# olga24912/lodestar

Hardware: AMD Instinct MI355X
Metric: verified signature sets/sec (node) (higher is better)
Workload: dtype u32/u64 (28-bit-limb Montgomery integer arithmetic); 1 GPU; C2 gossip attestation flood: 16384 single-pubkey sets per GPU, 1 set per batchable job; pk_mode=device table, sig_encoding=compressed 96 B, distinct_messages=16384, group_sets=1024, group_policy=0, inflight=32, slots=3, hw_queues=4, merge_sets=131072, pipeline_depth=3, parallelism=shard-by-job x1 (in-process devices), no collective

## Files before the change

### lodestar_amd/csrc/curve.hpp

```cpp
#pragma once
#include "tower.hpp"

BLS_HD fp F_add(const fp& a, const fp& b) { return fp_add(a, b); }
BLS_HD fp F_sub(const fp& a, const fp& b) { return fp_sub(a, b); }
BLS_HD fp F_mul(const fp& a, const fp& b) { return fp_mul(a, b); }
BLS_HD fp F_sqr(const fp& a) { return fp_sqr(a); }
BLS_HD fp F_dbl(const fp& a) { return fp_dbl(a); }
BLS_HD fp F_neg(const fp& a) { return fp_neg(a); }
BLS_HD bool F_is_zero(const fp& a) { return fp_is_zero(a); }
BLS_HD fp F_select(bool c, const fp& a, const fp& b) { return fp_select(c, a, b); }
BLS_HD fp F_add_nr(const fp& a, const fp& b) { return fp_add_nr(a, b); }
BLS_HD fp F_add_sq(const fp& a, const fp& b) { return fp_add_nr(a, b); }
BLS_HD fp2 F_add(const fp2& a, const fp2& b) { return fp2_add(a, b); }
BLS_HD fp2 F_sub(const fp2& a, const fp2& b) { return fp2_sub(a, b); }
BLS_HD fp2 F_mul(const fp2& a, const fp2& b) { return fp2_mul(a, b); }
BLS_HD fp2 F_sqr(const fp2& a) { return fp2_sqr(a); }
BLS_HD fp2 F_dbl(const fp2& a) { return fp2_dbl(a); }
BLS_HD fp2 F_neg(const fp2& a) { return fp2_neg(a); }
BLS_HD bool F_is_zero(const fp2& a) { return fp2_is_zero(a); }
BLS_HD fp2 F_select(bool c, const fp2& a, const fp2& b) { return fp2_select(c, a, b); }
BLS_HD fp2 F_add_nr(const fp2& a, const fp2& b) { return fp2_add_nr(a, b); }
BLS_HD fp2 F_add_sq(const fp2& a, const fp2& b) { return fp2_add_norm(a, b); }
template <int W, class F>
struct lt {
// ... 161 lines not shown
    if (F_is_zero(rr)) return jac_dbl(p);
    return jac_infinity<F>();
  }
  F HH = F_sqr(H);
  F I = F_dbl(F_dbl(HH));
  F J = F_mul(H, I);
  F V = F_mul(p.x, I);
  jac<F> r;
  r.x = F_sub(F_sub(F_sqr(rr), J), F_dbl(V));
  r.y = F_sub(F_mul(rr, F_sub(V, r.x)), F_dbl(F_mul(p.y, J)));
  r.z = F_sub(F_sub(F_sqr(F_add(p.z, H)), Z1Z1), HH);
  return r;
}
template <class F>
BLS_INL jac<F> jac_add_aff(const jac<F>& p, const aff<F>& q) {
  if constexpr (lazy_curve<F>::addaff)
    return jac_add_aff_lazy(p, q);
  else
    return jac_add_aff_eager(p, q);
}

template <class F>
BLS_INL jac<F> jac_add_lazy(const jac<F>& p, const jac<F>& q) {
  if (jac_is_inf(p)) return q;
  if (jac_is_inf(q)) return p;
  const F Z1Z1 = F_sqr(p.z);
  const F Z2Z2 = F_sqr(q.z);
  const F U1 = F_mul(p.x, Z2Z2);
  const F U2 = F_mul(q.x, Z1Z1);
  const F S1 = F_mul(p.y, F_mul(q.z, Z2Z2));
  const F S2 = F_mul(q.y, F_mul(p.z, Z1Z1));
  const F H = F_lc(L<1>(U2), L<-1>(U1));
  const F rr = F_lc(L<2>(S2), L<-2>(S1));
  if (F_is_zero(H)) {
    if (F_is_zero(rr)) return jac_dbl(p);
    return jac_infinity<F>();
  }
  const F I = F_sqr(F_add_sq(H, H));
  const F J = F_mul(H, I);
  const F V = F_mul(U1, I);
  const F R2 = F_sqr(rr);
  jac<F> r;
  r.x = F_lc(L<1>(R2), L<-1>(J), L<-2>(V));
  const F M = F_mul(rr, F_lc(L<3>(V), L<-1>(R2), L<1>(J)));
  const F N = F_mul(S1, J);
  r.y = F_lc(L<1>(M), L<-2>(N));
  r.z = F_mul(F_lc(L<1>(F_sqr(F_add_sq(p.z, q.z))), L<-1>(Z1Z1), L<-1>(Z2Z2)), H);
  return r;
}
template <class F>
BLS_INL jac<F> jac_add_eager(const jac<F>& p, const jac<F>& q) {
  if (jac_is_inf(p)) return q;
  if (jac_is_inf(q)) return p;
  F Z1Z1 = F_sqr(p.z);
  F Z2Z2 = F_sqr(q.z);
  F U1 = F_mul(p.x, Z2Z2);
  F U2 = F_mul(q.x, Z1Z1);
  F S1 = F_mul(p.y, F_mul(q.z, Z2Z2));
  F S2 = F_mul(q.y, F_mul(p.z, Z1Z1));
  F H = F_sub(U2, U1);
  F rr = F_dbl(F_sub(S2, S1));
  if (F_is_zero(H)) {
    if (F_is_zero(rr)) return jac_dbl(p);
    return jac_infinity<F>();
  }
  F I = F_sqr(F_dbl(H));
  F J = F_mul(H, I);
  F V = F_mul(U1, I);
  jac<F> r;
  r.x = F_sub(F_sub(F_sqr(rr), J), F_dbl(V));
  r.y = F_sub(F_mul(rr, F_sub(V, r.x)), F_dbl(F_mul(S1, J)));
  r.z = F_mul(F_sub(F_sub(F_sqr(F_add(p.z, q.z)), Z1Z1), Z2Z2), H);
  return r;
}
template <class F>
BLS_INL jac<F> jac_add(const jac<F>& p, const jac<F>& q) {
  if constexpr (lazy_curve<F>::add)
    return jac_add_lazy(p, q);
  else
    return jac_add_eager(p, q);
}

template <class F>
BLS_HDNI jac<F> jac_mul_u64(const aff<F>& P, uint64_t k) {
  jac<F> r = jac_infinity<F>();
  if (k == 0) return r;
  int top = 63;
  while (((k >> top) & 1ull) == 0) top--;
  r = jac_from_aff(P);
  for (int i = top - 1; i >= 0; i--) {
    r = jac_dbl(r);
    if ((k >> i) & 1ull) r = jac_add_aff(r, P);
  }
  return r;
}

template <class F>
BLS_HDNI jac<F> jac_mul_zabs(const jac<F>& P) {
  jac<F> r = P;
  for (int i = 62; i >= 0; i--) {
    r = jac_dbl(r);
    if ((BLS_Z_ABS >> i) & 1ull) r = jac_add(r, P);
  }
  return r;
}

template <class F, class LoadP>
BLS_INL jac<F> jac_mul_zabs_ld(LoadP loadP) {
  jac<F> r = loadP();
#pragma unroll 1
  for (int i = 62; i >= 0; i--) {
    r = jac_dbl(r);
    if ((BLS_Z_ABS >> i) & 1ull) r = jac_add(r, loadP());
  }
  return r;
}
template <class F, class LoadA>
BLS_INL jac<F> jac_mul_zabs_lda(LoadA loadA) {
  jac<F> r = jac_from_aff(loadA());
#pragma unroll 1
  for (int i = 62; i >= 0; i--) {
    r = jac_dbl(r);
    if ((BLS_Z_ABS >> i) & 1ull) r = jac_add_aff(r, loadA());
  }
  return r;
}

BLS_HDNI bool jac_to_aff(const g1j& p, g1a& out) {
  if (jac_is_inf(p)) return false;
  fp zi = fp_inv(p.z);
  fp zi2 = fp_sqr(zi);
  out.x = fp_mul(p.x, zi2);
  out.y = fp_mul(p.y, fp_mul(zi2, zi));
  return true;
}
BLS_HDNI bool jac_to_aff(const g2j& p, g2a& out) {
  if (jac_is_inf(p)) return false;
  fp2 zi = fp2_inv(p.z);
  fp2 zi2 = fp2_sqr(zi);
  out.x = fp2_mul(p.x, zi2);
  out.y = fp2_mul(p.y, fp2_mul(zi2, zi));
  return true;
}

template <class F>
BLS_FN bool jac_eq(const jac<F>& p, const jac<F>& q) {
  bool pi = jac_is_inf(p), qi = jac_is_inf(q);
  if (pi || qi) return pi && qi;
  F Z1Z1 = F_sqr(p.z), Z2Z2 = F_sqr(q.z);
  if (!F_is_zero(F_sub(F_mul(p.x, Z2Z2), F_mul(q.x, Z1Z1)))) return false;
  F a = F_mul(p.y, F_mul(q.z, Z2Z2));
  F b = F_mul(q.y, F_mul(p.z, Z1Z1));
  return F_is_zero(F_sub(a, b));
}

BLS_FN g2j g2_psi(const g2j& p) {
  g2j r;
  r.x = fp2_mul(fp2_conj(p.x), PSI_X);
  r.y = fp2_mul(fp2_conj(p.y), PSI_Y);
  r.z = fp2_conj(p.z);
  return r;
}
BLS_FN g2j g2_psi2(const g2j& p) {
  g2j r;
  r.x = fp2_mul(p.x, PSI2_X);
  r.y = fp2_mul(p.y, PSI2_Y);
  r.z = p.z;
  return r;
}

BLS_FN g1j endo_lambda(const g1j& p) {
  g1j r = p;
  r.x = fp_mul(p.x, G1_BETA);
  return r;
}
BLS_FN g2j endo_lambda(const g2j& p) { return jac_neg(g2_psi2(p)); }

BLS_HDNI bool g2_in_subgroup(const g2a& p) {
  g2j P = jac_from_aff(p);
  g2j zP = jac_neg(jac_mul_zabs(P));
  return jac_eq(g2_psi(P), zP);
}
template <class LoadA>
BLS_INL bool g2_in_subgroup_ld(LoadA loadA) {
  const g2j zP = jac_neg(jac_mul_zabs_lda<fp2>(loadA));
  return jac_eq(g2_psi(jac_from_aff(loadA())), zP);
}

BLS_HD bool g1_on_curve(const g1a& p) {
  return fp_eq(fp_sqr(p.y), fp_add(fp_mul(fp_sqr(p.x), p.x), FP_B1));
}
BLS_HD bool g2_on_curve(const g2a& p) {
  return fp2_eq(fp2_sqr(p.y), fp2_add(fp2_mul(fp2_sqr(p.x), p.x), FP2_B2));
}
```

### lodestar_amd/csrc/k_awr.hip

```cpp
#include "k_common.hpp"
#include "seg_sum.hpp"

BLS_INL int awr_point(const AwrBuffers& a, uint32_t k, g1j& P, bool& skip) {
  skip = false;
  g1a q;
  if (a.pk_bytes) {
    uint8_t raw[96];
    const uint4* src = reinterpret_cast<const uint4*>(a.pk_bytes + (size_t)k * 96);
#pragma unroll
    for (int c = 0; c < 6; c++) {
      const uint4 v = src[c];
      const uint32_t w[4] = {v.x, v.y, v.z, v.w};
#pragma unroll
      for (int j = 0; j < 16; j++) raw[16 * c + j] = (uint8_t)(w[j >> 2] >> (8 * (j & 3)));
    }
    bool inf = false;
    int st = pk_decode96(raw, q, inf);
    if (st == BLS_OK && inf) st = BLS_PK_IS_INFINITY;
    if (st != BLS_OK) return st;
  } else {
    const uint32_t idx = a.pk_index[k];
    if (idx >= a.pk_table_n) return BLS_DEVICE_ERROR;
    q = ld_pktab(a.pk_table, idx);
  }
  P = jac_from_aff(q);
  return BLS_OK;
}
BLS_INL int awr_point(const AwrBuffers& a, uint32_t k, g2j& P, bool& skip) {
  const int st = a.sig_status[k];
  skip = st == BLS_OK && (a.sig_flags[k] & SF_SIG_INF);
  if (st == BLS_OK && !skip) P = jac_from_aff(ld_g2a(a.sig_aff, a.n, k));
  return st;
}

template <class F>
BLS_INL void awr_strided(const AwrBuffers& a, uint32_t first, uint32_t last, uint32_t t, uint32_t L, uint32_t q,
                         jac<F>& acc, uint32_t& err_k, int& err) {
#pragma unroll 1
  for (uint32_t k = first + t; k < last; k += L) {
    jac<F> P;
    bool skip;
    const int st = awr_point(a, k, P, skip);
    if (st != BLS_OK) {
      if (err == 0) {
        err = st;
        err_k = k;
      }
      continue;
    }
    if (skip) continue;
    const uint32_t qq = opaque_u32(q);
    tab_st(a.tab, a.tab_n, qq, 8, acc);
    const jac<F> R = jac_mul_scalar_word(P, a.words[k], a.tab, a.tab_n, qq);
    acc = jac_add(tab_ld<F>(a.tab, a.tab_n, opaque_u32(q), 8), R);
  }
}

BLS_INL uint32_t* awr_sums(const AwrBuffers& a, const g1j*) { return a.sum_pk; }
BLS_INL uint32_t* awr_sums(const AwrBuffers& a, const g2j*) { return a.sum_sig; }
template <class F>
BLS_INL void awr_store(const AwrBuffers& a, uint32_t g, const jac<F>& acc, uint32_t err_k, int err) {
  constexpr int which = sizeof(F) == sizeof(fp) ? 0 : 1;
  uint32_t* o = awr_sums(a, (const jac<F>*)0);
  const uint32_t* s = reinterpret_cast<const uint32_t*>(&acc);
#pragma unroll
  for (int w = 0; w < (int)(sizeof(jac<F>) / 4); w++) o[(size_t)w * a.n_groups + g] = s[w];
  a.err_k[which * a.n_groups + g] = err_k;
  a.err_c[which * a.n_groups + g] = (int8_t)err;
}

template <class F, int L>
STAGE_KERNEL_W(1) void k_awr_sum(AwrBuffers a) {
  const uint32_t q = blockIdx.x * WAVE + threadIdx.x;
  const uint32_t t = q % L, g = q / L;
  const bool on = g < a.n_groups;
  const uint32_t first = on ? a.group_first[g] : 0, last = on ? a.group_first[g + 1] : 0;
  jac<F> acc = jac_infinity<F>();
  uint32_t my_err_k = 0xffffffffu;
  int my_err = 0;
  awr_strided<F>(a, first, last, t, L, q, acc, my_err_k, my_err);
  if constexpr (L == WAVE) {
    __shared__ uint32_t red[SEG_SLOTS * (sizeof(jac<F>) / 4)];
    __shared__ uint32_t err_k[WAVE];
    __shared__ int32_t err_c[WAVE];
    uint32_t bk;
    int bc;
    seg_wave_first_error(err_k, err_c, t, my_err_k, my_err, bk, bc);
    if (last - first > 1) seg_wave_tree(acc, red, t);
    my_err_k = bk;
    my_err = bc;
  } else {
    seg_butterfly<F, L>(acc, my_err_k, my_err);
  }
  if (on && t == 0) awr_store<F>(a, g, acc, my_err_k, my_err);
}

__global__ __launch_bounds__(WAVE) void k_awr_serialize(AwrBuffers a, uint8_t* out_pk, uint32_t out_pk_len,
                                                        uint8_t* out_sig, uint32_t out_sig_len, int8_t* status,
                                                        uint32_t* first_bad) {
  const uint32_t g = blockIdx.x * WAVE + threadIdx.x;
  if (g >= a.n_groups) return;
  const uint32_t kp = a.err_k[g], ks = a.err_k[a.n_groups + g];
  const bool key_first = kp <= ks;
  const uint32_t bad = key_first ? kp : ks;
  int st = key_first ? a.err_c[g] : a.err_c[a.n_groups + g];
  if (a.group_first[g + 1] == a.group_first[g]) st = BLS_EMPTY_AGGREGATE;
  uint8_t buf[192];
  for (int k = 0; k < 192; k++) buf[k] = 0;
  if (st == BLS_OK) {
    g1a p;
    if (!jac_to_aff(ld_g1j(a.sum_pk, a.n_groups, g), p)) {
      buf[0] = out_pk_len == 48 ? 0xc0 : 0x40;
    } else if (out_pk_len == 48) {
      g1a_compress(p, buf);
    } else {
      g1a_to_be96(p, buf);
    }
  }
  uint8_t* o = out_pk + (size_t)g * out_pk_len;
  for (uint32_t k = 0; k < out_pk_len; k++) o[k] = buf[k];
  for (int k = 0; k < 96; k++) buf[k] = 0;
  if (st == BLS_OK) {
    g2a s;
    if (!jac_to_aff(ld_g2j(a.sum_sig, a.n_groups, g), s)) {
      buf[0] = out_sig_len == 96 ? 0xc0 : 0x40;
    } else if (out_sig_len == 96) {
      g2a_compress(s, buf);
    } else {
      g2a_to_be192(s, buf);
    }
  }
  o = out_sig + (size_t)g * out_sig_len;
  for (uint32_t k = 0; k < out_sig_len; k++) o[k] = buf[k];
  status[g] = (int8_t)st;
  first_bad[g] = st == BLS_OK || st == BLS_EMPTY_AGGREGATE ? 0xffffffffu : bad;
}
// ... 32 lines not shown
```

### lodestar_amd/csrc/k_common.hpp

```cpp
#pragma once
#include <atomic>

#include "kernels.h"
#include "ops.hpp"
#include "fp2x.hpp"

#define WAVE 64
#if defined(__HIP_DEVICE_COMPILE__) && !BLS_INLINE_PRODUCTS && !BLS_FP2_CLASSIC
static_assert(WAVE <= BLS_FP2_LDS_LANES, "fp2_mul LDS slot");
static_assert(2 * WAVE <= BLS_FP2_LDS_LANES, "128-lane kernels (gt_wave.hpp, k_msm_bucket) and fp2_mul LDS slot");
#endif

#ifndef BLSGPU_WPE
#define BLSGPU_WPE 1
#endif
#define STAGE_KERNEL __global__ __launch_bounds__(WAVE) __attribute__((amdgpu_waves_per_eu(BLSGPU_WPE, BLSGPU_WPE)))
#define STAGE_KERNEL_W(w) __global__ __launch_bounds__(WAVE) __attribute__((amdgpu_waves_per_eu(w, w)))
#ifndef BLSGPU_WPE_PK
#define BLSGPU_WPE_PK BLSGPU_WPE
#endif
#ifndef BLSGPU_WPE_HPREP
#define BLSGPU_WPE_HPREP 1
#endif
#ifndef BLSGPU_WPE_MSM
#define BLSGPU_WPE_MSM BLSGPU_WPE
#endif
#ifndef BLSGPU_WPE_LINES
#define BLSGPU_WPE_LINES BLSGPU_WPE
#endif
#ifndef BLSGPU_WPE_ACC
#define BLSGPU_WPE_ACC BLSGPU_WPE
#endif
#ifndef BLSGPU_WPE_DEC
#define BLSGPU_WPE_DEC BLSGPU_WPE
#endif
#ifndef BLSGPU_WPE_HASH
#define BLSGPU_WPE_HASH BLSGPU_WPE
#endif
#ifndef BLSGPU_WPE_HMAP
#define BLSGPU_WPE_HMAP 2
#endif
#ifndef BLSGPU_WPE_GRP
#define BLSGPU_WPE_GRP BLSGPU_WPE
#endif

__device__ __forceinline__ uint32_t opaque_u32(uint32_t x) {
  asm volatile("" : "+v"(x));
  return x;
}

__device__ __forceinline__ fp ld_fp(const uint32_t* p, uint32_t n, uint32_t i, int w0) {
  fp r;
#pragma unroll
  for (int l = 0; l < BLS_NL; l++) r.l[l] = p[(size_t)(w0 + l) * n + i];
  return r;
}
__device__ __forceinline__ void st_fp(uint32_t* p, uint32_t n, uint32_t i, int w0, const fp& v) {
#pragma unroll
  for (int l = 0; l < BLS_NL; l++) p[(size_t)(w0 + l) * n + i] = v.l[l];
}
__device__ __forceinline__ fp2 ld_fp2(const uint32_t* p, uint32_t n, uint32_t i, int w0) {
  return fp2_make(ld_fp(p, n, i, w0), ld_fp(p, n, i, w0 + W_FP));
}
__device__ __forceinline__ void st_fp2(uint32_t* p, uint32_t n, uint32_t i, int w0, const fp2& v) {
  st_fp(p, n, i, w0, v.c0);
  st_fp(p, n, i, w0 + W_FP, v.c1);
}
__device__ __forceinline__ g2a ld_g2a(const uint32_t* p, uint32_t n, uint32_t i) {
  g2a r;
  r.x = ld_fp2(p, n, i, 0);
  r.y = ld_fp2(p, n, i, 2 * W_FP);
  return r;
}
__device__ __forceinline__ void st_g2a(uint32_t* p, uint32_t n, uint32_t i, const g2a& v) {
  st_fp2(p, n, i, 0, v.x);
  st_fp2(p, n, i, 2 * W_FP, v.y);
}
__device__ __forceinline__ g2j ld_g2j(const uint32_t* p, uint32_t n, uint32_t i) {
  g2j r;
  r.x = ld_fp2(p, n, i, 0);
  r.y = ld_fp2(p, n, i, 2 * W_FP);
  r.z = ld_fp2(p, n, i, 4 * W_FP);
  return r;
}
__device__ __forceinline__ void st_g2j(uint32_t* p, uint32_t n, uint32_t i, const g2j& v) {
  st_fp2(p, n, i, 0, v.x);
  st_fp2(p, n, i, 2 * W_FP, v.y);
  st_fp2(p, n, i, 4 * W_FP, v.z);
}
__device__ __forceinline__ g1a ld_g1a(const uint32_t* p, uint32_t n, uint32_t i) {
  g1a r;
  r.x = ld_fp(p, n, i, 0);
  r.y = ld_fp(p, n, i, W_FP);
  return r;
}
__device__ __forceinline__ void st_g1a(uint32_t* p, uint32_t n, uint32_t i, const g1a& v) {
  st_fp(p, n, i, 0, v.x);
  st_fp(p, n, i, W_FP, v.y);
}
__device__ __forceinline__ g1j ld_g1j(const uint32_t* p, uint32_t n, uint32_t i) {
  g1j r;
  r.x = ld_fp(p, n, i, 0);
// ... 55 lines not shown
  for (int s = 0; s < MILLER_STEPS; s++) {
    line3 L;
    if (!add_next) {
      miller_dbl_line(T, L);
      add_next = (BLS_Z_ABS >> bit) & 1ull;
      bit--;
    } else {
      miller_add_line(T, Q, L);
      add_next = false;
    }
    uint32_t* o = lines + (size_t)s * W_LINE * nm;
    st_fp2(o, nm, u, 0, L.l0);
    st_fp2(o, nm, u, 2 * W_FP, L.c1);
    st_fp2(o, nm, u, 4 * W_FP, L.c4);
  }
}

BLS_INL fp fp_shfl(const fp& x, int src) {
  fp r;
#pragma unroll
  for (int i = 0; i < BLS_NL; i++) r.l[i] = (uint32_t)__shfl((int)x.l[i], src);
  return r;
}
BLS_INL fp2 fp2_shfl(const fp2& x, int src) { return fp2_make(fp_shfl(x.c0, src), fp_shfl(x.c1, src)); }
BLS_INL fp fp_keep(bool c, const fp& a) { return fp_select(c, a, fp_zero()); }
#define ACC6_GROUPS (WAVE / 6)
BLS_INL g2j g2j_xlane(const g2j& p) {
  g2j r;
  r.x = fp2_xlane(p.x);
  r.y = fp2_xlane(p.y);
  r.z = fp2_xlane(p.z);
  return r;
}
__device__ __forceinline__ g1a ld_pktab(const uint32_t* tab, uint32_t idx) {
  const uint4* q = reinterpret_cast<const uint4*>(tab + (size_t)idx * W_PKTAB);
  uint32_t w[W_PKTAB];
#pragma unroll
  for (int k = 0; k < W_PKTAB / 4; k++) {
    uint4 v = q[k];
    w[4 * k] = v.x;
    w[4 * k + 1] = v.y;
    w[4 * k + 2] = v.z;
    w[4 * k + 3] = v.w;
  }
  g1a r;
#pragma unroll
  for (int l = 0; l < BLS_NL; l++) {
    r.x.l[l] = w[l];
    r.y.l[l] = w[BLS_NL + l];
  }
  return r;
}

template <class F>
__device__ jac<F> jac_mul_u64_j(const jac<F>& P, uint64_t k) {
  jac<F> r = jac_infinity<F>();
  if (k == 0) return r;
  int top = 63;
  while (((k >> top) & 1ull) == 0) top--;
  r = P;
  for (int i = top - 1; i >= 0; i--) {
    r = jac_dbl(r);
    if ((k >> i) & 1ull) r = jac_add(r, P);
  }
  return r;
}

template <class F>
__device__ __forceinline__ void tab_st(uint32_t* tab, uint32_t n, uint32_t i, int e, const jac<F>& v) {
  constexpr int WF = sizeof(F) / 4;
  const uint32_t* s = reinterpret_cast<const uint32_t*>(&v);
#pragma unroll
  for (int w = 0; w < 3 * WF; w++) tab[((size_t)e * 3 * WF + w) * n + i] = s[w];
}
template <class F>
__device__ __forceinline__ jac<F> tab_ld(const uint32_t* tab, uint32_t n, uint32_t i, int e) {
  constexpr int WF = sizeof(F) / 4;
  jac<F> v;
  uint32_t* d = reinterpret_cast<uint32_t*>(&v);
#pragma unroll
  for (int w = 0; w < 3 * WF; w++) d[w] = tab[((size_t)e * 3 * WF + w) * n + i];
  return v;
}
BLS_HD int scalar_word_digit(uint64_t w, int k, bool& neg) {
  const int d = 2 * (int)((w >> (4 * k)) & 15u) - 15;
  neg = d < 0;
  return (d < 0 ? -d : d) >> 1;
}
template <class F>
__device__ jac<F> jac_mul_scalar_word(const jac<F>& P, uint64_t w, uint32_t* tab, uint32_t n, uint32_t i) {
  const jac<F> P2 = jac_dbl(P);
  jac<F> t = P;
  tab_st(tab, n, i, 0, t);
#pragma unroll 1
  for (int e = 1; e < 8; e++) {
    t = jac_add(t, P2);
    tab_st(tab, n, i, e, t);
  }
  const uint32_t ii = opaque_u32(i);
  auto term = [&](int k, bool hi) {
    bool neg;
    const int e = scalar_word_digit(w, hi ? k + 8 : k, neg);
    jac<F> q = tab_ld<F>(tab, n, ii, e);
    if (hi) q = endo_lambda(q);
    return neg ? jac_neg(q) : q;
  };
  jac<F> r = jac_add(term(7, false), term(7, true));
#pragma unroll 1
  for (int k = 6; k >= 0; k--) {
    r = jac_dbl(jac_dbl(jac_dbl(jac_dbl(r))));
    r = jac_add(r, term(k, false));
    r = jac_add(r, term(k, true));
  }
  return r;
}

template <class F>
__device__ jac<F> jac_mul_words(const jac<F>& P, const uint32_t* k, int nw) {
  jac<F> r = jac_infinity<F>();
  for (int i = 32 * nw - 1; i >= 0; i--) {
    r = jac_dbl(r);
    if ((k[i >> 5] >> (i & 31)) & 1u) r = jac_add(r, P);
  }
  return r;
}


template <auto kernel>
inline size_t exclusive_cu_lds() {
  constexpr int kMaxDev = 64;
  static std::atomic<int64_t> cache[kMaxDev];
  int dev = 0;
  if (hipGetDevice(&dev) != hipSuccess || dev < 0 || dev >= kMaxDev) return 0;
  const int64_t c = cache[dev].load(std::memory_order_acquire);
  if (c) return (size_t)(c - 1);
  const size_t pad = [&]() -> size_t {
    int max_block = 0, per_cu = 0;
    if (hipDeviceGetAttribute(&max_block, hipDeviceAttributeMaxSharedMemoryPerBlock, dev) != hipSuccess) return 0;
    if (hipDeviceGetAttribute(&per_cu, hipDeviceAttributeMaxSharedMemoryPerMultiprocessor, dev) != hipSuccess)
      return 0;
    hipFuncAttributes a{};
    if (hipFuncGetAttributes(&a, reinterpret_cast<const void*>(kernel)) != hipSuccess) return 0;
    const size_t want = (size_t)per_cu - 8 * 1024;
    if (per_cu <= 0 || (size_t)max_block < want || a.sharedSizeBytes >= want) return 0;
    const size_t pad_b = want - a.sharedSizeBytes;
    if (hipFuncSetAttribute(reinterpret_cast<const void*>(kernel), hipFuncAttributeMaxDynamicSharedMemorySize,
                            (int)pad_b) != hipSuccess)
      return 0;
    return pad_b;
  }();
  cache[dev].store((int64_t)pad + 1, std::memory_order_release);
  return pad;
}
```

### lodestar_amd/csrc/k_pk.hip

```cpp
#include "k_common.hpp"
#include "pk_row.hpp"

static_assert(PK_ROW_WORDS == W_PKTAB, "pk_row.hpp restates the row width of kernels.h");

#ifndef BLSGPU_PK_AGG_GROUPS
#define BLSGPU_PK_AGG_GROUPS 1
#endif
__global__ __launch_bounds__(WAVE) void k_pk_aggregate(PipelineBuffers b, uint32_t n_sets) {
  __shared__ uint32_t red[WAVE * W_G1J];
  __shared__ uint32_t err_k[WAVE];
  __shared__ int32_t err_c[WAVE];
  if (blockIdx.x >= n_sets) return;
  const uint32_t set = b.agg_sets ? b.agg_sets[blockIdx.x] : blockIdx.x;
  uint32_t lane = threadIdx.x;
  int8_t* agg_status = b.status + 2 * b.n;
  const uint32_t first = b.set_pk_first[set], last = b.set_pk_first[set + 1];
  g1j acc = jac_infinity<fp>();
  uint32_t my_err_k = 0xffffffffu;
  int my_err = 0;
  for (uint32_t k = first + lane; k < last; k += WAVE) {
    g1a q;
    if (b.pk_bytes) {
      uint8_t raw[96];
      const uint8_t* src = b.pk_bytes + (size_t)k * 96;
// ... 93 lines not shown
      const int st = pk_decode96(raw, pt, inf);
      if (st != BLS_OK) {
        if (my_err == 0) {
          my_err = st;
          my_err_k = k;
        }
        continue;
      }
      if (inf) continue;
    } else {
      const uint32_t idx = b.pk_index[k];
      if (idx >= b.pk_table_n) {
        if (my_err == 0) {
          my_err = BLS_DEVICE_ERROR;
          my_err_k = k;
        }
        continue;
      }
      pt = ld_pktab(b.pk_table, idx);
    }
    acc = jac_add_aff(acc, pt);
  }
#pragma unroll 1
  for (int m = L / 2; m >= 1; m >>= 1) {
    g1j o;
    o.x = fp_shfl_xor(acc.x, m);
    o.y = fp_shfl_xor(acc.y, m);
    o.z = fp_shfl_xor(acc.z, m);
    const uint32_t ok = (uint32_t)__shfl_xor((int)my_err_k, m);
    const int oc = __shfl_xor(my_err, m);
    if (ok < my_err_k) {
      my_err_k = ok;
      my_err = oc;
    }
    acc = jac_add(acc, o);
  }
  if (on && t == 0) {
    b.status[2 * b.n + set] = (int8_t)my_err;
    st_g1j(b.pk_jac, b.n, set, acc);
  }
}

__device__ __forceinline__ int set_pubkey(const PipelineBuffers& b, uint32_t i, g1j& P) {
  const bool one = b.set_pk_first && b.pk_direct1 && b.set_pk_first[i + 1] - b.set_pk_first[i] == 1;
  if (one && !b.pk_bytes) {
    const uint32_t idx = b.pk_index[b.set_pk_first[i]];
    if (idx >= b.pk_table_n) return BLS_DEVICE_ERROR;
    P = jac_from_aff(ld_pktab(b.pk_table, idx));
    return BLS_OK;
  }
  if (b.pk_bytes && (!b.set_pk_first || one)) {
    uint8_t raw[96];
    const uint32_t k = b.set_pk_first ? b.set_pk_first[i] : i;
    const uint4* src = reinterpret_cast<const uint4*>(b.pk_bytes + (size_t)k * 96);
#pragma unroll
    for (int k = 0; k < 6; k++) {
      uint4 v = src[k];
      uint32_t w[4] = {v.x, v.y, v.z, v.w};
#pragma unroll
      for (int j = 0; j < 16; j++) raw[16 * k + j] = (uint8_t)(w[j >> 2] >> (8 * (j & 3)));
    }
    g1a a;
    bool inf = false;
    int st = pk_decode96(raw, a, inf);
    if (st == BLS_OK && inf) st = BLS_PK_IS_INFINITY;
    if (st == BLS_OK) P = jac_from_aff(a);
    return st;
  }
  if (b.set_pk_first[i + 1] == b.set_pk_first[i]) return BLS_EMPTY_AGGREGATE;
  const int st = b.status[2 * b.n + i];
  if (st) return st;
  P = ld_g1j(b.pk_jac, b.n, i);
  return jac_is_inf(P) ? BLS_PK_IS_INFINITY : BLS_OK;
}

STAGE_KERNEL_W(BLSGPU_WPE_PK) void k_pk_finish(PipelineBuffers b, uint32_t n_sets, int8_t* pk_status) {
  uint32_t i = blockIdx.x * WAVE + threadIdx.x;
  if (i >= n_sets) return;
  g1j P;
  int st = set_pubkey(b, i, P);
  g1j R = jac_infinity<fp>();
  if (st == BLS_OK) {
    const uint64_t w = b.scalars[i];
    R = (w == 0) ? P : jac_mul_scalar_word(P, w, b.scal_tab, b.n, i);
  }
  st_g1j(b.pk_jac, b.n, i, R);
  pk_status[i] = (int8_t)st;
}

STAGE_KERNEL void k_unit_aggregate(PipelineBuffers b) {
  uint32_t u = blockIdx.x * WAVE + threadIdx.x;
  if (u >= b.n_units) return;
  const uint32_t a = b.unit_set_first[u], e = b.unit_set_first[u + 1];
  g1a out;
  out.x = fp_zero();
  out.y = fp_zero();
  bool ok = false;
  if (e - a == 1) {
    const uint32_t i = b.unit_sets[a];
    if (b.include[i]) {
      out = ld_g1a(b.pk_aff, b.n, i);
      ok = true;
    }
  } else {
    g1j acc = jac_infinity<fp>();
    for (uint32_t k = a; k < e; k++) {
      const uint32_t i = b.unit_sets[k];
      if (b.include[i]) acc = jac_add_aff(acc, ld_g1a(b.pk_aff, b.n, i));
    }
    ok = jac_to_aff(acc, out);
  }
  st_g1a(b.unit_p, b.n, u, out);
  b.unit_ok[u] = ok ? 1 : 0;
}

__global__ __launch_bounds__(WAVE) void k_pk_serialize(PipelineBuffers b, uint32_t n_sets, uint8_t* out,
                                                       uint32_t out_len) {
  uint32_t i = blockIdx.x * WAVE + threadIdx.x;
  if (i >= n_sets) return;
  int st = b.set_pk_first[i + 1] == b.set_pk_first[i] ? BLS_EMPTY_AGGREGATE : b.status[2 * b.n + i];
  uint8_t buf[96];
  for (int k = 0; k < 96; k++) buf[k] = 0;
  if (st == BLS_OK) {
    g1a a;
    if (!jac_to_aff(ld_g1j(b.pk_jac, b.n, i), a)) {
      buf[0] = out_len == 48 ? 0xc0 : 0x40;
    } else if (out_len == 48) {
      g1a_compress(a, buf);
    } else {
      g1a_to_be96(a, buf);
    }
  }
  uint8_t* o = out + (size_t)i * out_len;
  for (uint32_t k = 0; k < out_len; k++) o[k] = buf[k];
  b.status[i] = (int8_t)st;
}

__global__ __launch_bounds__(WAVE) void k_key_validate(const uint8_t* pks, uint32_t n, uint32_t pk_len, uint32_t stride,
                                                       uint8_t* out96, int8_t* status) {
  uint32_t i = blockIdx.x * WAVE + threadIdx.x;
  if (i >= n) return;
  uint8_t raw[96];
  const uint8_t* src = pks + (size_t)i * stride;
  for (uint32_t k = 0; k < 96; k++) raw[k] = k < pk_len ? src[k] : 0;
  g1a a;
  const int st = pk_key_validate(raw, pk_len, a);
  uint8_t buf[96];
  for (int k = 0; k < 96; k++) buf[k] = 0;
  if (st == BLS_OK) g1a_to_be96(a, buf);
  if (out96)
    for (int k = 0; k < 96; k++) out96[(size_t)i * 96 + k] = buf[k];
  status[i] = (int8_t)st;
}

__global__ __launch_bounds__(WAVE) void k_pk_table_fill(const uint8_t* pk96, uint32_t n, uint32_t* table_dst,
                                                        int8_t* status) {
  uint32_t i = blockIdx.x * WAVE + threadIdx.x;
  if (i >= n) return;
  uint8_t raw[96];
  for (int k = 0; k < 96; k++) raw[k] = pk96[(size_t)i * 96 + k];
  g1a a;
  bool inf = false;
  int st = pk_decode96(raw, a, inf);
  if (st == BLS_OK && inf) st = BLS_PK_IS_INFINITY;
  uint32_t* dst = table_dst + (size_t)i * W_PKTAB;
  for (int l = 0; l < BLS_NL; l++) {
    dst[l] = st == BLS_OK ? a.x.l[l] : 0;
    dst[BLS_NL + l] = st == BLS_OK ? a.y.l[l] : 0;
  }
  dst[2 * BLS_NL] = 0;
  dst[2 * BLS_NL + 1] = 0;
  dst[2 * BLS_NL + 2] = 0;
  dst[2 * BLS_NL + 3] = 0;
  status[i] = (int8_t)st;
}

template <bool validate>
__global__ __launch_bounds__(WAVE) void k_pk_table_fill48(const uint8_t* pk48, uint32_t n, uint32_t* table_dst,
                                                          int8_t* status) {
  const uint32_t i = blockIdx.x * WAVE + threadIdx.x;
  if (i >= n) return;
  uint8_t raw[48];
  const uint4* src = reinterpret_cast<const uint4*>(pk48 + (size_t)i * 48);
#pragma unroll
  for (int k = 0; k < 3; k++) {
    const uint4 v = src[k];
    const uint32_t w[4] = {v.x, v.y, v.z, v.w};
#pragma unroll
    for (int j = 0; j < 16; j++) raw[16 * k + j] = (uint8_t)(w[j >> 2] >> (8 * (j & 3)));
  }
  uint32_t row[W_PKTAB];
  const int st = pk_row_from48<validate>(raw, row);
  uint4* dst = reinterpret_cast<uint4*>(table_dst + (size_t)i * W_PKTAB);
#pragma unroll
  for (int k = 0; k < W_PKTAB / 4; k++) dst[k] = make_uint4(row[4 * k], row[4 * k + 1], row[4 * k + 2], row[4 * k + 3]);
  status[i] = (int8_t)st;
}

__global__ __launch_bounds__(WAVE) void k_pk_table_read(const uint32_t* table, uint32_t first, uint32_t n, uint8_t* out,
                                                        uint32_t out_len) {
  const uint32_t i = blockIdx.x * WAVE + threadIdx.x;
  if (i >= n) return;
  const g1a a = ld_pktab(table, first + i);
  uint8_t buf[96];
  pk_point_to_bytes(a, out_len, buf);
  uint4* dst = reinterpret_cast<uint4*>(out + (size_t)i * out_len);
  const uint32_t quads = out_len / 16;
#pragma unroll
  for (uint32_t k = 0; k < 6; k++) {
    if (k >= quads) break;
    uint32_t w[4];
#pragma unroll
    for (int j = 0; j < 4; j++)
      w[j] = (uint32_t)buf[16 * k + 4 * j] | (uint32_t)buf[16 * k + 4 * j + 1] << 8 |
             (uint32_t)buf[16 * k + 4 * j + 2] << 16 | (uint32_t)buf[16 * k + 4 * j + 3] << 24;
    dst[k] = make_uint4(w[0], w[1], w[2], w[3]);
  }
}

static inline dim3 grid_for(uint32_t n) { return dim3((n + WAVE - 1) / WAVE); }

void launch_pk_aggregate(const PipelineBuffers& b, uint32_t n, hipStream_t s) {
  if (b.agg_sets) n = b.n_agg;
  if (!n) return;
  const uint32_t lanes = 1024 * WAVE;
  if ((uint64_t)n * 64 <= lanes || !BLSGPU_PK_AGG_GROUPS)
    hipLaunchKernelGGL(k_pk_aggregate, dim3(n), dim3(WAVE), 0, s, b, n);
  else if ((uint64_t)n * 32 <= 2 * lanes)
    hipLaunchKernelGGL(k_pk_aggregate_g<32>, dim3((n * 32 + WAVE - 1) / WAVE), dim3(WAVE), 0, s, b, n);
  else if ((uint64_t)n * 16 <= 2 * lanes)
    hipLaunchKernelGGL(k_pk_aggregate_g<16>, dim3((n * 16 + WAVE - 1) / WAVE), dim3(WAVE), 0, s, b, n);
  else
    hipLaunchKernelGGL(k_pk_aggregate_g<8>, dim3((n * 8 + WAVE - 1) / WAVE), dim3(WAVE), 0, s, b, n);
}
void launch_pk_finish(const PipelineBuffers& b, uint32_t n, hipStream_t s) {
  if (n) hipLaunchKernelGGL(k_pk_finish, grid_for(n), dim3(WAVE), 0, s, b, n, b.status + b.n);
}
void launch_unit_aggregate(const PipelineBuffers& b, hipStream_t s) {
  if (b.n_units) hipLaunchKernelGGL(k_unit_aggregate, grid_for(b.n_units), dim3(WAVE), 0, s, b);
}
void launch_pk_serialize(const PipelineBuffers& b, uint32_t n, uint8_t* out, uint32_t out_len, hipStream_t s) {
  if (n) hipLaunchKernelGGL(k_pk_serialize, grid_for(n), dim3(WAVE), 0, s, b, n, out, out_len);
}
void launch_key_validate(const uint8_t* pks, uint32_t n, uint32_t pk_len, uint32_t stride, uint8_t* out96,
                         int8_t* status, hipStream_t s) {
  if (n) hipLaunchKernelGGL(k_key_validate, grid_for(n), dim3(WAVE), 0, s, pks, n, pk_len, stride, out96, status);
}
void launch_pk_table_fill(const uint8_t* pk96, uint32_t n, uint32_t* table_dst, int8_t* status, hipStream_t s) {
  if (n) hipLaunchKernelGGL(k_pk_table_fill, grid_for(n), dim3(WAVE), 0, s, pk96, n, table_dst, status);
}
void launch_pk_table_fill48(const uint8_t* pk48, uint32_t n, uint32_t* table_dst, int8_t* status, bool validate,
                            hipStream_t s) {
  if (!n) return;
  if (validate)
    hipLaunchKernelGGL(k_pk_table_fill48<true>, grid_for(n), dim3(WAVE), 0, s, pk48, n, table_dst, status);
  else
    hipLaunchKernelGGL(k_pk_table_fill48<false>, grid_for(n), dim3(WAVE), 0, s, pk48, n, table_dst, status);
}
void launch_pk_table_read(const uint32_t* table, uint32_t first, uint32_t n, uint8_t* out, uint32_t out_len,
                          hipStream_t s) {
  if (n) hipLaunchKernelGGL(k_pk_table_read, grid_for(n), dim3(WAVE), 0, s, table, first, n, out, out_len);
}
```

### lodestar_amd/csrc/k_sig.hip

```cpp
#include "k_common.hpp"
#include "g2_coop.hpp"

#ifndef BLSGPU_SIG_PAIRS
#define BLSGPU_SIG_PAIRS 1
#endif
#ifndef BLSGPU_WPE_DEC0
#define BLSGPU_WPE_DEC0 2
#endif
#ifndef BLSGPU_WPE_SUB2
#define BLSGPU_WPE_SUB2 2
#endif
template <bool CHECK, int WPE>
__global__ __launch_bounds__(WAVE) __attribute__((amdgpu_waves_per_eu(WPE, WPE))) void k_sig_decode(
    PipelineBuffers b, uint32_t n_sets) {
  const bool check_group = CHECK;
  uint32_t i = blockIdx.x * WAVE + threadIdx.x;
  if (i >= n_sets) return;
  uint8_t raw[192];
  uint32_t len = b.sig_len[i];
  const uint8_t* src = b.sigs + (size_t)i * b.sig_stride;
  uint32_t cl = len == 96 || len == 192 ? len : 0;
  for (uint32_t k = 0; k < cl; k++) raw[k] = src[k];
  g2a p;
  bool inf = false;
  int st = sig_decode_point(raw, len, p, inf);
  if (st != BLS_OK || inf) {
    p.x = fp2_zero();
    p.y = fp2_zero();
  }
  st_g2a(b.sig_aff, b.n, i, p);
  if (check_group && st == BLS_OK && !inf &&
      !g2_in_subgroup_ld([&] { return ld_g2a(b.sig_aff, b.n, opaque_u32(i)); })) {
    st = BLS_POINT_NOT_IN_GROUP;
    p.x = fp2_zero();
    p.y = fp2_zero();
    st_g2a(b.sig_aff, b.n, i, p);
  }
  b.flags[i] = inf ? SF_SIG_INF : 0;
  b.status[i] = (int8_t)st;
}

STAGE_KERNEL_W(BLSGPU_WPE_SUB2) void k_sig_subgroup2(PipelineBuffers b, uint32_t n_sets) {
  const uint32_t q = blockIdx.x * WAVE + threadIdx.x, i = q >> 1, k = q & 1;
  if (i >= n_sets || b.status[i] != BLS_OK || (b.flags[i] & SF_SIG_INF)) return;
  auto ldP = [&] {
    const uint32_t ii = opaque_u32(i);
    aff<fp2x> a;
    a.x.v = ld_fp(b.sig_aff, b.n, ii, (int)(k * W_FP));
    a.y.v = ld_fp(b.sig_aff, b.n, ii, (int)((2 + k) * W_FP));
    return a;
  };
  const g2jx zP = jac_neg(jac_mul_zabs_lda<fp2x>(ldP));
  if (!jac_eq(g2_psi(jac_from_aff(ldP())), zP)) {
    st_fp(b.sig_aff, b.n, i, (int)(k * W_FP), fp_zero());
    st_fp(b.sig_aff, b.n, i, (int)((2 + k) * W_FP), fp_zero());
    if (k == 0) b.status[i] = (int8_t)BLS_POINT_NOT_IN_GROUP;
  }
}

STAGE_KERNEL void k_sig_scale(PipelineBuffers b, uint32_t n_sets, const uint32_t* list) {
  const uint32_t q = blockIdx.x * WAVE + threadIdx.x;
  if (q >= n_sets) return;
  const uint32_t i = list ? list[q] : q;
  g2j R = jac_infinity<fp2>();
  if (b.status[i] == BLS_OK && !(b.flags[i] & SF_SIG_INF)) {
    const g2a s = ld_g2a(b.sig_aff, b.n, i);
    const uint64_t w = b.scalars[i];
    R = (w == 0) ? jac_from_aff(s) : jac_mul_scalar_word(jac_from_aff(s), w, b.scal_tab, b.n, i);
  }
  st_g2j(b.rsig, b.n, i, R);
}

#define SG_GROUPS (WAVE / G2C_LANES)
__global__ __launch_bounds__(WAVE) void k_sig_subgroup_coop(PipelineBuffers b, uint32_t n_sets) {
  __shared__ uint32_t lds[SG_GROUPS * G2C_WORDS];
  const uint32_t tg = threadIdx.x % G2C_LANES, grp = threadIdx.x / G2C_LANES;
  const uint32_t i = blockIdx.x * SG_GROUPS + grp;
  uint32_t* g = lds + grp * G2C_WORDS;
  const bool on = i < n_sets && b.status[i] == BLS_OK && !(b.flags[i] & SF_SIG_INF);
  if (tg == 0 && on) g2c_st_point(g, jac_from_aff(ld_g2a(b.sig_aff, b.n, i)));
  g2c_sync();
  g2c_mul_zabs(g, tg, on, [&] { return jac_from_aff(ld_g2a(b.sig_aff, b.n, opaque_u32(i))); });
  if (tg == 0 && on) {
    const g2j zP = jac_neg(g2c_ld_point(g));
    if (!jac_eq(g2_psi(jac_from_aff(ld_g2a(b.sig_aff, b.n, i))), zP)) {
      g2a z;
      z.x = fp2_zero();
      z.y = fp2_zero();
      st_g2a(b.sig_aff, b.n, i, z);
      b.status[i] = (int8_t)BLS_POINT_NOT_IN_GROUP;
    }
  }
}

__global__ __launch_bounds__(WAVE) void k_spec_mask(PipelineBuffers b, uint32_t n_sets, uint8_t* spec) {
  const uint32_t i = blockIdx.x * WAVE + threadIdx.x;
  if (i < n_sets) spec[i] = b.status[i] == BLS_OK ? 1 : 0;
}

static inline dim3 grid_for(uint32_t n) { return dim3((n + WAVE - 1) / WAVE); }

void launch_spec_mask(const PipelineBuffers& b, uint32_t n, uint8_t* spec, hipStream_t s) {
  if (n) hipLaunchKernelGGL(k_spec_mask, grid_for(n), dim3(WAVE), 0, s, b, n, spec);
}

void launch_sig_decode(const PipelineBuffers& b, uint32_t n, hipStream_t s, bool coop, hipEvent_t decoded,
                       bool exclusive, bool subgroup) {
  if (!n) return;
  if (!subgroup) {
    hipLaunchKernelGGL((k_sig_decode<false, BLSGPU_WPE_DEC0>), grid_for(n), dim3(WAVE), 0, s, b, n);
    if (decoded) (void)hipEventRecord(decoded, s);
    return;
  }
  if (coop || BLSGPU_SIG_PAIRS)
    hipLaunchKernelGGL((k_sig_decode<false, BLSGPU_WPE_DEC0>), grid_for(n), dim3(WAVE), 0, s, b, n);
  else
    hipLaunchKernelGGL((k_sig_decode<true, BLSGPU_WPE_DEC>), grid_for(n), dim3(WAVE), 0, s, b, n);
  if (decoded) (void)hipEventRecord(decoded, s);
  if (!coop) {
    if (BLSGPU_SIG_PAIRS) hipLaunchKernelGGL(k_sig_subgroup2, grid_for(2 * n), dim3(WAVE), 0, s, b, n);
  } else
    hipLaunchKernelGGL(k_sig_subgroup_coop, dim3((n + SG_GROUPS - 1) / SG_GROUPS), dim3(WAVE),
                       BLSGPU_EXCLUSIVE_SMALL && exclusive ? exclusive_cu_lds<k_sig_subgroup_coop>() : 0, s, b, n);
}
void launch_sig_scale(const PipelineBuffers& b, uint32_t n, hipStream_t s, const uint32_t* list) {
  if (n) hipLaunchKernelGGL(k_sig_scale, grid_for(n), dim3(WAVE), 0, s, b, n, list);
}
```

Baseline: 4.321 million sets/s.

## Use co-Z affine precomputation table for scalar-word multiplication with deferred general fallback

```diff
diff --git a/lodestar_amd/csrc/curve.hpp b/lodestar_amd/csrc/curve.hpp
--- a/lodestar_amd/csrc/curve.hpp
+++ b/lodestar_amd/csrc/curve.hpp
@@ -267,6 +267,39 @@
 }
 
 template <class F>
+BLS_FN void jac_dbl_upd(const jac<F>& p, jac<F>& d, aff<F>& u) {
+  const F A = F_sqr(p.x);
+  const F B = F_sqr(p.y);
+  const F C = F_sqr(B);
+  const F S = F_sqr(F_add_sq(p.x, B));
+  u.x = F_lc(L<2>(S), L<-2>(A), L<-2>(C));
+  u.y = F_lc(L<8>(C));
+  const F E = F_lc(L<3>(A));
+  const F Fv = F_sqr(E);
+  d.x = F_lc(L<1>(Fv), L<-2>(u.x));
+  const F M = F_mul(E, F_lc(L<3>(u.x), L<-1>(Fv)));
+  d.y = F_lc(L<1>(M), L<-1>(u.y));
+  d.z = F_mul(F_add_nr(p.y, p.y), p.z);
+}
+template <class F>
+BLS_FN aff<F> aff_add_coz_upd(aff<F>& a, const aff<F>& b, F& h) {
+  h = F_lc(L<1>(a.x), L<-1>(b.x));
+  const F c = F_sqr(h);
+  const F W1 = F_mul(a.x, c);
+  const F W2 = F_mul(b.x, c);
+  const F dy = F_lc(L<1>(a.y), L<-1>(b.y));
+  const F d = F_sqr(dy);
+  const F A1 = F_mul(a.y, F_lc(L<1>(W1), L<-1>(W2)));
+  aff<F> r;
+  r.x = F_lc(L<1>(d), L<-1>(W1), L<-1>(W2));
+  const F M = F_mul(dy, F_lc(L<2>(W1), L<1>(W2), L<-1>(d)));
+  r.y = F_lc(L<1>(M), L<-1>(A1));
+  a.x = W1;
+  a.y = A1;
+  return r;
+}
+
+template <class F>
 BLS_HDNI jac<F> jac_mul_u64(const aff<F>& P, uint64_t k) {
   jac<F> r = jac_infinity<F>();
   if (k == 0) return r;
@@ -360,6 +393,17 @@
   return r;
 }
 BLS_FN g2j endo_lambda(const g2j& p) { return jac_neg(g2_psi2(p)); }
+BLS_FN g1a endo_lambda(const g1a& p) {
+  g1a r = p;
+  r.x = fp_mul(p.x, G1_BETA);
+  return r;
+}
+BLS_FN g2a endo_lambda(const g2a& p) {
+  g2a r;
+  r.x = fp2_mul(p.x, PSI2_X);
+  r.y = fp2_neg(fp2_mul(p.y, PSI2_Y));
+  return r;
+}
 
 BLS_HDNI bool g2_in_subgroup(const g2a& p) {
   g2j P = jac_from_aff(p);
diff --git a/lodestar_amd/csrc/k_awr.hip b/lodestar_amd/csrc/k_awr.hip
--- a/lodestar_amd/csrc/k_awr.hip
+++ b/lodestar_amd/csrc/k_awr.hip
@@ -51,7 +51,7 @@
     if (skip) continue;
     const uint32_t qq = opaque_u32(q);
     tab_st(a.tab, a.tab_n, qq, 8, acc);
-    const jac<F> R = jac_mul_scalar_word(P, a.words[k], a.tab, a.tab_n, qq);
+    const jac<F> R = jac_mul_scalar_word_jacobian(P, a.words[k], a.tab, a.tab_n, qq);
     acc = jac_add(tab_ld<F>(a.tab, a.tab_n, opaque_u32(q), 8), R);
   }
 }
diff --git a/lodestar_amd/csrc/k_common.hpp b/lodestar_amd/csrc/k_common.hpp
--- a/lodestar_amd/csrc/k_common.hpp
+++ b/lodestar_amd/csrc/k_common.hpp
@@ -4,6 +4,7 @@
 #include "kernels.h"
 #include "ops.hpp"
 #include "fp2x.hpp"
+#include "scalar_word.hpp"
 
 #define WAVE 64
 #if defined(__HIP_DEVICE_COMPILE__) && !BLS_INLINE_PRODUCTS && !BLS_FP2_CLASSIC
@@ -17,7 +18,7 @@
 #define STAGE_KERNEL __global__ __launch_bounds__(WAVE) __attribute__((amdgpu_waves_per_eu(BLSGPU_WPE, BLSGPU_WPE)))
 #define STAGE_KERNEL_W(w) __global__ __launch_bounds__(WAVE) __attribute__((amdgpu_waves_per_eu(w, w)))
 #ifndef BLSGPU_WPE_PK
-#define BLSGPU_WPE_PK BLSGPU_WPE
+#define BLSGPU_WPE_PK 2
 #endif
 #ifndef BLSGPU_WPE_HPREP
 #define BLSGPU_WPE_HPREP 1
@@ -239,13 +240,56 @@
   for (int w = 0; w < 3 * WF; w++) d[w] = tab[((size_t)e * 3 * WF + w) * n + i];
   return v;
 }
-BLS_HD int scalar_word_digit(uint64_t w, int k, bool& neg) {
-  const int d = 2 * (int)((w >> (4 * k)) & 15u) - 15;
-  neg = d < 0;
-  return (d < 0 ? -d : d) >> 1;
-}
+template <class F, bool Deferred>
+struct hbm_scalar_tab {
+  uint32_t* tab;
+  uint32_t n, i;
+  uint32_t ii;
+  static constexpr int WF = sizeof(F) / 4;
+  __device__ __forceinline__ void st(int e, int c, const F& v) {
+    const uint32_t* s = reinterpret_cast<const uint32_t*>(&v);
+#pragma unroll
+    for (int w = 0; w < WF; w++) tab[((size_t)(e * 3 + c) * WF + w) * n + i] = s[w];
+  }
+  __device__ __forceinline__ F ld(int e, int c) const {
+    F v;
+    uint32_t* d = reinterpret_cast<uint32_t*>(&v);
+#pragma unroll
+    for (int w = 0; w < WF; w++) d[w] = tab[((size_t)(e * 3 + c) * WF + w) * n + ii];
+    return v;
+  }
+  __device__ __forceinline__ void stj(int e, const jac<F>& v) { tab_st(tab, n, i, e, v); }
+  __device__ __forceinline__ jac<F> ldj(int e) const { return tab_ld<F>(tab, n, ii, e); }
+  __device__ __forceinline__ void reads() { ii = opaque_u32(i); }
+  __device__ __forceinline__ jac<F> general(uint64_t w) {
+    if constexpr (Deferred)
+      return jac_infinity<F>();
+    else
+      return jac_mul_scalar_word_general_in<F>(w, *this);
+  }
+};
 template <class F>
 __device__ jac<F> jac_mul_scalar_word(const jac<F>& P, uint64_t w, uint32_t* tab, uint32_t n, uint32_t i) {
+  hbm_scalar_tab<F, false> t{tab, n, i, i};
+  return jac_mul_scalar_word_coz(P, w, t, (bool*)nullptr);
+}
+template <class F>
+__device__ jac<F> jac_mul_scalar_word_deferred(const jac<F>& P, uint64_t w, uint32_t* tab, uint32_t n, uint32_t i) {
+  hbm_scalar_tab<F, true> t{tab, n, i, i};
+  return jac_mul_scalar_word_coz(P, w, t, (bool*)nullptr);
+}
+template <class F>
+__device__ __forceinline__ bool scalar_word_pending(uint32_t* tab, uint32_t n, uint32_t i) {
+  hbm_scalar_tab<F, true> t{tab, n, i, i};
+  return F_is_zero(t.ld(6, 2));
+}
+template <class F>
+__device__ jac<F> jac_mul_scalar_word_general(uint64_t w, uint32_t* tab, uint32_t n, uint32_t i) {
+  hbm_scalar_tab<F, false> t{tab, n, i, i};
+  return jac_mul_scalar_word_general_in<F>(w, t);
+}
+template <class F>
+__device__ jac<F> jac_mul_scalar_word_jacobian(const jac<F>& P, uint64_t w, uint32_t* tab, uint32_t n, uint32_t i) {
   const jac<F> P2 = jac_dbl(P);
   jac<F> t = P;
   tab_st(tab, n, i, 0, t);
diff --git a/lodestar_amd/csrc/k_pk.hip b/lodestar_amd/csrc/k_pk.hip
--- a/lodestar_amd/csrc/k_pk.hip
+++ b/lodestar_amd/csrc/k_pk.hip
@@ -199,10 +199,19 @@
   g1j R = jac_infinity<fp>();
   if (st == BLS_OK) {
     const uint64_t w = b.scalars[i];
-    R = (w == 0) ? P : jac_mul_scalar_word(P, w, b.scal_tab, b.n, i);
+    R = (w == 0) ? P : jac_mul_scalar_word_deferred(P, w, b.scal_tab, b.n, i);
   }
   st_g1j(b.pk_jac, b.n, i, R);
   pk_status[i] = (int8_t)st;
+}
+#define PK_GENERAL_WAVES 64
+STAGE_KERNEL void k_pk_finish_general(PipelineBuffers b, uint32_t n_sets, const int8_t* pk_status) {
+#pragma unroll 1
+  for (uint32_t i = blockIdx.x * WAVE + threadIdx.x; i < n_sets; i += gridDim.x * WAVE) {
+    const uint64_t w = b.scalars[i];
+    if (pk_status[i] != BLS_OK || w == 0 || !scalar_word_pending<fp>(b.scal_tab, b.n, i)) continue;
+    st_g1j(b.pk_jac, b.n, i, jac_mul_scalar_word_general<fp>(w, b.scal_tab, b.n, i));
+  }
 }
 
 STAGE_KERNEL void k_unit_aggregate(PipelineBuffers b) {
@@ -351,7 +360,11 @@
     hipLaunchKernelGGL(k_pk_aggregate_g<8>, dim3((n * 8 + WAVE - 1) / WAVE), dim3(WAVE), 0, s, b, n);
 }
 void launch_pk_finish(const PipelineBuffers& b, uint32_t n, hipStream_t s) {
-  if (n) hipLaunchKernelGGL(k_pk_finish, grid_for(n), dim3(WAVE), 0, s, b, n, b.status + b.n);
+  if (!n) return;
+  hipLaunchKernelGGL(k_pk_finish, grid_for(n), dim3(WAVE), 0, s, b, n, b.status + b.n);
+  const uint32_t waves = (n + WAVE - 1) / WAVE;
+  hipLaunchKernelGGL(k_pk_finish_general, dim3(waves < PK_GENERAL_WAVES ? waves : PK_GENERAL_WAVES), dim3(WAVE), 0, s, b, n,
+                     b.status + b.n);
 }
 void launch_unit_aggregate(const PipelineBuffers& b, hipStream_t s) {
   if (b.n_units) hipLaunchKernelGGL(k_unit_aggregate, grid_for(b.n_units), dim3(WAVE), 0, s, b);
diff --git a/lodestar_amd/csrc/k_sig.hip b/lodestar_amd/csrc/k_sig.hip
--- a/lodestar_amd/csrc/k_sig.hip
+++ b/lodestar_amd/csrc/k_sig.hip
@@ -66,9 +66,20 @@
   if (b.status[i] == BLS_OK && !(b.flags[i] & SF_SIG_INF)) {
     const g2a s = ld_g2a(b.sig_aff, b.n, i);
     const uint64_t w = b.scalars[i];
-    R = (w == 0) ? jac_from_aff(s) : jac_mul_scalar_word(jac_from_aff(s), w, b.scal_tab, b.n, i);
+    R = (w == 0) ? jac_from_aff(s) : jac_mul_scalar_word_deferred(jac_from_aff(s), w, b.scal_tab, b.n, i);
   }
   st_g2j(b.rsig, b.n, i, R);
+}
+#define SIG_GENERAL_WAVES 64
+STAGE_KERNEL void k_sig_scale_general(PipelineBuffers b, uint32_t n_sets, const uint32_t* list) {
+#pragma unroll 1
+  for (uint32_t q = blockIdx.x * WAVE + threadIdx.x; q < n_sets; q += gridDim.x * WAVE) {
+    const uint32_t i = list ? list[q] : q;
+    const uint64_t w = b.scalars[i];
+    if (b.status[i] != BLS_OK || (b.flags[i] & SF_SIG_INF) || w == 0) continue;
+    if (!scalar_word_pending<fp2>(b.scal_tab, b.n, i)) continue;
+    st_g2j(b.rsig, b.n, i, jac_mul_scalar_word_general<fp2>(w, b.scal_tab, b.n, i));
+  }
 }
 
 #define SG_GROUPS (WAVE / G2C_LANES)
@@ -124,5 +135,9 @@
                        BLSGPU_EXCLUSIVE_SMALL && exclusive ? exclusive_cu_lds<k_sig_subgroup_coop>() : 0, s, b, n);
 }
 void launch_sig_scale(const PipelineBuffers& b, uint32_t n, hipStream_t s, const uint32_t* list) {
-  if (n) hipLaunchKernelGGL(k_sig_scale, grid_for(n), dim3(WAVE), 0, s, b, n, list);
+  if (!n) return;
+  hipLaunchKernelGGL(k_sig_scale, grid_for(n), dim3(WAVE), 0, s, b, n, list);
+  const uint32_t waves = (n + WAVE - 1) / WAVE;
+  hipLaunchKernelGGL(k_sig_scale_general, dim3(waves < SIG_GENERAL_WAVES ? waves : SIG_GENERAL_WAVES), dim3(WAVE), 0, s, b, n,
+                     list);
 }
diff --git a/lodestar_amd/csrc/scalar_word.hpp b/lodestar_amd/csrc/scalar_word.hpp
--- /dev/null
+++ b/lodestar_amd/csrc/scalar_word.hpp
@@ -0,0 +1,101 @@
+#pragma once
+#include "curve.hpp"
+
+BLS_HD int scalar_word_digit(uint64_t w, int k, bool& neg) {
+  const int d = 2 * (int)((w >> (4 * k)) & 15u) - 15;
+  neg = d < 0;
+  return (d < 0 ? -d : d) >> 1;
+}
+
+template <class F, class Tab>
+BLS_INL jac<F> jac_mul_scalar_word_jac(const jac<F>& P, uint64_t w, Tab& tab) {
+  const jac<F> P2 = jac_dbl(P);
+  jac<F> t = P;
+  tab.stj(0, t);
+#pragma unroll 1
+  for (int e = 1; e < 8; e++) {
+    t = jac_add(t, P2);
+    tab.stj(e, t);
+  }
+  tab.reads();
+  auto term = [&](int k, bool hi) {
+    bool neg;
+    const int e = scalar_word_digit(w, hi ? k + 8 : k, neg);
+    jac<F> q = tab.ldj(e);
+    if (hi) q = endo_lambda(q);
+    return neg ? jac_neg(q) : q;
+  };
+  jac<F> r = jac_add(term(7, false), term(7, true));
+#pragma unroll 1
+  for (int k = 6; k >= 0; k--) {
+    r = jac_dbl(jac_dbl(jac_dbl(jac_dbl(r))));
+    r = jac_add(r, term(k, false));
+    r = jac_add(r, term(k, true));
+  }
+  return r;
+}
+
+template <class F, class Tab>
+BLS_INL jac<F> jac_mul_scalar_word_general_in(uint64_t w, Tab& tab) {
+  jac<F> Q;
+  Q.x = tab.ld(0, 0), Q.y = tab.ld(0, 1), Q.z = tab.ld(7, 2);
+  return jac_mul_scalar_word_jac(Q, w, tab);
+}
+
+template <class F, class Tab>
+BLS_INL jac<F> jac_mul_scalar_word_coz(const jac<F>& P, uint64_t w, Tab& tab, bool* general) {
+  {
+    jac<F> D;
+    aff<F> t;
+    jac_dbl_upd(P, D, t);
+    tab.st(7, 2, D.z);
+    tab.st(0, 0, t.x), tab.st(0, 1, t.y);
+    aff<F> d;
+    d.x = D.x, d.y = D.y;
+#pragma unroll 1
+    for (int e = 1; e < 8; e++) {
+      F h;
+      t = aff_add_coz_upd(d, t, h);
+      tab.st(e - 1, 2, h);
+      tab.st(e, 0, t.x), tab.st(e, 1, t.y);
+    }
+  }
+  tab.reads();
+  F s = tab.ld(6, 2);
+#pragma unroll 1
+  for (int j = 6; j > 0; j--) {
+    const F s2 = F_sqr(s);
+    tab.st(j, 0, F_mul(tab.ld(j, 0), s2));
+    tab.st(j, 1, F_mul(tab.ld(j, 1), F_mul(s2, s)));
+    s = F_mul(s, tab.ld(j - 1, 2));
+  }
+  const F zt = F_mul(tab.ld(7, 2), s);
+  const bool exc = F_is_zero(zt);
+  tab.st(6, 2, zt);
+  if (general) *general = exc;
+  if (exc) return tab.general(w);
+  {
+    const F s2 = F_sqr(s);
+    tab.st(0, 0, F_mul(tab.ld(0, 0), s2));
+    tab.st(0, 1, F_mul(tab.ld(0, 1), F_mul(s2, s)));
+  }
+  auto term = [&](int k, bool hi) {
+    bool neg;
+    const int e = scalar_word_digit(w, hi ? k + 8 : k, neg);
+    aff<F> q;
+    q.x = tab.ld(e, 0), q.y = tab.ld(e, 1);
+    if (hi) q = endo_lambda(q);
+    if (neg) q.y = F_neg(q.y);
+    return q;
+  };
+  jac<F> r = jac_add_aff(jac_from_aff(term(7, false)), term(7, true));
+#pragma unroll 1
+  for (int k = 6; k >= 0; k--) {
+    r = jac_dbl(jac_dbl(jac_dbl(jac_dbl(r))));
+    r = jac_add_aff(r, term(k, false));
+    r = jac_add_aff(r, term(k, true));
+  }
+  tab.reads();
+  r.z = F_mul(r.z, tab.ld(6, 2));
+  return r;
+}
```

Result: slower. 4.205 million sets/s (-2.7%).
